# bluecube/minipath

Hardware: AMD Instinct MI355X
Metric: Mrays/s (higher is better)
Workload: dtype f32

## Files before the change

### minipath_amd/csrc/kernels.hip

```cpp
#include <hip/hip_runtime.h>

#include <algorithm>
#include <cfloat>
#include <cmath>
#include <cstdlib>
#include <type_traits>

#include "launch_plan.h"
#include "mp_internal.h"
#include "family_launch.h"
#include "ray_math.h"

#ifdef MP_PROF_MISSES
namespace mp {
namespace {
__device__ unsigned long long g_prof[8];
}
}
#define MP_PROF_COUNT(i) do { if ((threadIdx.x & 63u) == 0u) atomicAdd(&g_prof[i], 1ull); } while (0)
#endif
#include "mask_cache.h"
#include "group_walk.h"

namespace mp {
namespace {

struct RenderParams {
    DevScene scene;
    RayGen gen;
    const mp_block* tiles;
    uint32_t n_tiles, tile_size;
    float* out;
    uint32_t* counter;
    float inv_spp;
    uint32_t s_begin, s_end;
    uint32_t carry_in;
    uint32_t finalize;
    uint32_t chunked;
    const uint32_t* tile_order;
    unsigned long long* tile_cost;
    uint32_t lds_per_wave;
    uint32_t max_depth;
    unsigned long long* segments;
    float* pool;
    uint32_t pool_stride;
};

constexpr uint32_t kSumChunk = 256;
__device__ __forceinline__ void pixel_state_load(const RenderParams& P, size_t off, bool inpix, bool writer, float& acc, float& cnt) {
    acc = 0.0f;
    cnt = 0.0f;
    if (P.carry_in && inpix) {
        const float4 prev = *reinterpret_cast<const float4*>(P.out + off);
        acc = prev.x;
        cnt = P.chunked ? prev.y : prev.w;
    } else if (P.chunked && inpix && writer) {
        *reinterpret_cast<double*>(P.out + off + 2) = 0.0;
    }
}
__device__ __forceinline__ void chunk_flush(const RenderParams& P, size_t off, bool writer, float& acc) {
    if (writer) {
        double* t = reinterpret_cast<double*>(P.out + off + 2);
        *t = *t + static_cast<double>(acc);
    }
    acc = 0.0f;
}
__device__ __forceinline__ void pixel_state_store(const RenderParams& P, size_t off, float acc, float cnt) {
    if (P.chunked) {
        if (!P.finalize) {
            *reinterpret_cast<float2*>(P.out + off) = make_float2(acc, cnt);
            return;
        }
// ... 284 lines not shown
                const bool det_ok = fabsf(det) <= kHuge;
                const float xu = det_ok ? as_f(as_u(un) ^ det_sign) : 1.0f;
                if (__ballot(!(xu <= thr)) == 0) return;
                const float qx = fms(sy, e1z, sz * e1y), qy = fms(sz, e1x, sx * e1z), qz = fms(sx, e1y, sy * e1x);
                const float vn = fma_dot(r.dx, r.dy, r.dz, qx, qy, qz);
                const float tn = fma_dot(e2x, e2y, e2z, qx, qy, qz);
                const float xv = det_ok ? as_f(as_u(vn) ^ det_sign) : 1.0f, xt = det_ok ? as_f(as_u(tn) ^ det_sign) : 1.0f;
                if (__ballot(!(fminf(fminf(xu, xv), xt) <= thr)) == 0) return;
                const float inv_det = 1.0f / det;
                const float u = inv_det * un, v = inv_det * vn, t = inv_det * tn;
                const bool acc = (u >= 0.0f) & (v >= 0.0f) & ((u + v) <= 1.0f) & (t >= 0.0f) & (t < lim);
                best_t = acc ? t : best_t;
                lim = acc ? t : lim;
                bu = acc ? u : bu;
                bv = acc ? v : bv;
                bprim = acc ? tri : bprim;
                changed |= __ballot(acc);
            };
            float a0 = tp[0], a1 = tp[1], a2 = tp[2], a3 = tp[3], a4 = tp[4], a5 = tp[5], a6 = tp[6], a7 = tp[7], a8 = tp[8];
            uint32_t tri = first * 8u;
            for (uint32_t p = n_real >> 1; p > 0; p--) {
                const float b0 = tp[9], b1 = tp[10], b2 = tp[11], b3 = tp[12], b4 = tp[13], b5 = tp[14], b6 = tp[15], b7 = tp[16], b8 = tp[17];
                test(a0, a1, a2, a3, a4, a5, a6, a7, a8, tri);
                a0 = tp[18]; a1 = tp[19]; a2 = tp[20]; a3 = tp[21]; a4 = tp[22]; a5 = tp[23]; a6 = tp[24]; a7 = tp[25]; a8 = tp[26];
                test(b0, b1, b2, b3, b4, b5, b6, b7, b8, tri + 1u);
                tri += 2u;
                tp += 2 * kTriDwords;
            }
            if (n_real & 1u) test(a0, a1, a2, a3, a4, a5, a6, a7, a8, tri);
            if (changed != 0) stale_top = sp;
        }
    }
    hit.t = best_t; hit.u = bu; hit.v = bv; hit.prim = bprim;
}

struct RegStack3 {
    int ent, mlo, mhi;
    __device__ __forceinline__ RegStack3() : ent(0), mlo(0), mhi(0) {}
    __device__ __forceinline__ void push(int sp, uint32_t e, uint64_t m) {
        asm volatile("s_mov_b32 m0, %3\n\ts_nop 0\n\t"
                     "v_writelane_b32 %0, %4, m0\n\tv_writelane_b32 %1, %5, m0\n\tv_writelane_b32 %2, %6, m0"
                     : "+v"(ent), "+v"(mlo), "+v"(mhi)
                     : "s"(sp), "s"(e), "s"(static_cast<uint32_t>(m)), "s"(static_cast<uint32_t>(m >> 32))
                     : "m0");
    }
    __device__ __forceinline__ void pop(int sp, uint32_t& e, uint64_t& m) const {
        e = static_cast<uint32_t>(__builtin_amdgcn_readlane(ent, sp));
        m = static_cast<uint32_t>(__builtin_amdgcn_readlane(mlo, sp)) |
            (static_cast<uint64_t>(static_cast<uint32_t>(__builtin_amdgcn_readlane(mhi, sp))) << 32);
    }
};

template <int OCT>
__device__ __noinline__ uint32_t unit_list_slow(const float* __restrict__ nodes_pk, uint32_t* mcache, uint32_t node, uint32_t slots) {
    return unit_list_build(reinterpret_cast<const float4*>(nodes_pk), mcache, node, slots,
                           [](const float* b, const float bmn[3], const float bmx[3]) { return bounds_may_hit<OCT>(b, bmn, bmx); });
}
template <int OCT>
__device__ __forceinline__ bool trace_packet_cached(const DevScene& sc, const Ray& r, bool active, PacketHit& hit, uint32_t* mcache) {
    static_assert(kNullLink == MP_LINK_NULL, "mask_cache.h's copy of the null link");
    kfp nodes = (kfp)(uintptr_t)sc.nodes_pk;
    kfp tris = (kfp)(uintptr_t)sc.tris_aos;
    float best_t = FLT_MAX, bu = 0.0f, bv = 0.0f;
    uint32_t bprim = kNoPrim;
    RegStack3 st;
    int sp = 0;
    mcache[kRootListSlot] = sc.pk_count * sc.pk_mask_bits;
    wave_lds_sync();
    uint32_t cur = (static_cast<uint32_t>(kRootListSlot) << 16) | 1u;
    uint64_t pm = __ballot(active);
    for (;;) {
        if ((cur & 0xFFFFu) == 0u) {
            if (sp == 0) break;
            sp--;
            st.pop(sp, cur, pm);
        }
        cur -= 1u;
        const uint32_t src = __builtin_amdgcn_readfirstlane(mcache[(cur >> 16) + (cur & 0xFFFFu)]);
#ifndef MP_NO_EMPTY_SKIP
        if (static_cast<int32_t>(src) < 0) {
            MP_PROF_COUNT(7);
            continue;
        }
#endif
        const bool pon = __builtin_amdgcn_inverse_ballot_w64(pm);
        const krec8 rec = *reinterpret_cast<const __attribute__((address_space(4))) krec8*>(reinterpret_cast<const __attribute__((address_space(4))) char*>(nodes) + scalar_u(src * 32u));
        float t1, t2;
        slab<false, OCT>(rec[0], rec[1], rec[2], rec[3], rec[4], rec[5], r, pon ? best_t : -1.0f, t1, t2);
        const bool ok = t1 <= t2;
        if (__ballot(ok) == 0) continue;
        const uint32_t link = uniform_u(rec[6]);
        float lim = ok ? best_t : -1.0f;
        if ((link & 63u) == 0u) {
            MP_PROF_COUNT(2);
            const uint32_t node = link >> 6;
            const uint32_t slot = node_slot(node);
            const uint32_t tag = __builtin_amdgcn_readfirstlane(mcache[static_cast<uint32_t>(kMaskCacheHeader) + slot]);
            uint32_t list = __builtin_amdgcn_readfirstlane(mcache[static_cast<uint32_t>(kNodeListBase) + slot]);
            if (__builtin_expect(tag != node, 0)) {
                MP_PROF_COUNT(0);
                if (tag != 0xFFFFFFFFu) MP_PROF_COUNT(4);
                list = __builtin_amdgcn_readfirstlane(unit_list_slow<OCT>(sc.nodes_pk, mcache, node, sc.pk_mask_bits));
                if (list == kListOverflow) {
                    if (sp != 0 || (cur & 0xFFFFu) != 0u) {
                        MP_PROF_COUNT(6);
                        return false;
                    }
                    list = __builtin_amdgcn_readfirstlane(unit_list_slow<OCT>(sc.nodes_pk, mcache, node, sc.pk_mask_bits));
                }
            }
            if ((list & 0xFFFFu) != 0u) {
                if ((cur & 0xFFFFu) != 0u) {
                    st.push(sp, cur, pm);
                    sp++;
                }
                cur = list;
                pm = __ballot(lim >= 0.0f);
            }
        } else {
            const uint32_t first = link >> 6, n_real = link & 63u;
            kfp tp = tris + static_cast<size_t>(first) * (8 * kTriDwords);
            static_assert(kExitTiny == kTiny && kExitHuge == kHuge, "mask_cache.h's copies of the early-out constants");
            const float thr = lim >= 0.0f ? -kTiny : INFINITY;
            auto test = [&](const float v0x, const float v0y, const float v0z, const float e1x, const float e1y, const float e1z,
                            const float e2x, const float e2y, const float e2z, const uint32_t tri) {
                const float hx = fms(r.dy, e2z, r.dz * e2y), hy = fms(r.dz, e2x, r.dx * e2z), hz = fms(r.dx, e2y, r.dy * e2x);
                const float det = fma_dot(e1x, e1y, e1z, hx, hy, hz);
                const float sx = r.ox - v0x, sy = r.oy - v0y, sz = r.oz - v0z;
                const float un = fma_dot(sx, sy, sz, hx, hy, hz);
                const float xu = tri_flipped(det, un);
                if (__ballot(!(tri_exit1_key(det, xu) <= thr)) == 0) return;
                const float qx = fms(sy, e1z, sz * e1y), qy = fms(sz, e1x, sx * e1z), qz = fms(sx, e1y, sy * e1x);
                const float vn = fma_dot(r.dx, r.dy, r.dz, qx, qy, qz);
                const float tn = fma_dot(e2x, e2y, e2z, qx, qy, qz);
                const float xv = tri_flipped(det, vn), xt = tri_flipped(det, tn);
                if (__ballot(!(tri_exit2_key(det, xu, xv, xt) <= thr)) == 0) return;
                constexpr uint32_t kRcpLo = 0x10800000u , kRcpHi = 0x7E000000u ;
                const uint32_t wkey = (as_u(det) << 1) - (kRcpLo << 1);
                const float inv_det = __ballot(wkey > ((kRcpHi - kRcpLo) << 1)) == 0 ? rm::rcp_short(det) : 1.0f / det;
                const float u = inv_det * un, v = inv_det * vn, t = inv_det * tn;
                const bool acc = !(fminf(fminf(u, v), t) < 0.0f) & ((u + v) <= 1.0f) & (t < lim);
                best_t = acc ? t : best_t;
                lim = acc ? t : lim;
                bu = acc ? u : bu;
                bv = acc ? v : bv;
                bprim = acc ? tri : bprim;
            };
            const uint32_t ls = first & static_cast<uint32_t>(kLeafCacheEntries - 1);
            const uint32_t tag = mcache[kLeafTagBase + ls];
            const uint2 tm = reinterpret_cast<const uint2*>(mcache + kLeafMaskBase)[ls];
            uint64_t todo;
            if (__builtin_expect(__builtin_amdgcn_readfirstlane(tag) == first, 1)) {
                todo = __builtin_amdgcn_readfirstlane(tm.x) | (static_cast<uint64_t>(__builtin_amdgcn_readfirstlane(tm.y)) << 32);
            } else {
                MP_PROF_COUNT(1);
                const uint64_t m = leaf_mask_slow(sc.tris_aos, mcache, first, n_real);
                todo = __builtin_amdgcn_readfirstlane(static_cast<uint32_t>(m)) | (static_cast<uint64_t>(__builtin_amdgcn_readfirstlane(static_cast<uint32_t>(m >> 32))) << 32);
            }
#ifndef MP_NO_EMPTY_SKIP
            if (todo == 0 && (cur >> 16) != static_cast<uint32_t>(kRootListSlot)) {
                if ((threadIdx.x & 63u) == 0u) mcache[(cur >> 16) + (cur & 0xFFFFu)] = src | kEmptyLeafBit;
                wave_lds_sync();
            }
#endif
            if (todo != 0) {
                uint32_t c = static_cast<uint32_t>(__builtin_ctzll(todo));
                todo &= ~(1ull << c);
                kfp ta = tri_record(tp, c);
                krec8 ra = *reinterpret_cast<const __attribute__((address_space(4))) krec8*>(ta);
                float a8 = ta[8];
                while (todo != 0) {
                    const uint32_t cn = static_cast<uint32_t>(__builtin_ctzll(todo));
                    todo &= ~(1ull << cn);
                    kfp tb = tri_record(tp, cn);
                    const krec8 rb = *reinterpret_cast<const __attribute__((address_space(4))) krec8*>(tb);
                    const float b8 = tb[8];
                    test(ra[0], ra[1], ra[2], ra[3], ra[4], ra[5], ra[6], ra[7], a8, first * 8u + c);
                    ra = rb; a8 = b8;
                    c = cn;
                }
                test(ra[0], ra[1], ra[2], ra[3], ra[4], ra[5], ra[6], ra[7], a8, first * 8u + c);
            }
        }
    }
    hit.t = best_t; hit.u = bu; hit.v = bv; hit.prim = bprim;
    return true;
}

template <bool OCTANTS, class Stack, bool MC = false>
__device__ __forceinline__ void trace_packet(const DevScene& sc, const Ray& r, bool active, Stack& st, PacketHit& hit,
                                             const MaskCache& mc = MaskCache{nullptr}) {
    if (OCTANTS && MC) {
        if (__ballot(active & !mask_cache_ray_ok(r)) != 0) {
            const bool slow = active && (fabsf(r.ix) == INFINITY || fabsf(r.iy) == INFINITY || fabsf(r.iz) == INFINITY);
            if (__ballot(slow) != 0) trace_packet_impl<2, -1>(sc, r, active, st, hit);
            else trace_packet_impl<1, -1>(sc, r, active, st, hit);
            return;
        }
    } else {
        const bool slow = active && (fabsf(r.ix) == INFINITY || fabsf(r.iy) == INFINITY || fabsf(r.iz) == INFINITY);
        if (__ballot(slow) != 0) {
            trace_packet_impl<2, -1>(sc, r, active, st, hit);
            return;
        }
    }
    if (OCTANTS && sc.boxes_ordered) {
        const uint64_t am = __ballot(active);
        const uint64_t nx = __ballot(active && r.ix < 0.0f), ny = __ballot(active && r.iy < 0.0f), nz = __ballot(active && r.iz < 0.0f);
// ... 1524 lines not shown
    (void)hipFreeAsync(ws, st);
    return rc;
}

int launch_trace_rays(const DevScene& sc, const float* ox, const float* oy, const float* oz, const float* dx,
                      const float* dy, const float* dz, uint64_t n, const mp_hits_soa& hits, int cu_count, void* stream,
                      std::string& err) {
    return launch_rays(kQueryClosest, sc, ox, oy, oz, dx, dy, dz, nullptr, n, &hits, nullptr, cu_count, stream, err);
}

int launch_query_rays(const DevScene& sc, const float* ox, const float* oy, const float* oz, const float* dx, const float* dy,
                      const float* dz, const float* tmax, uint64_t n, const mp_hits_soa* hits, uint8_t* occluded, int cu_count,
                      void* stream, std::string& err) {
    return launch_rays(occluded ? kQueryAnyHit : kQueryBounded, sc, ox, oy, oz, dx, dy, dz, tmax, n, hits, occluded, cu_count, stream, err);
}

int launch_set_u64(unsigned long long* d_ptr, unsigned long long value, void* stream, std::string& err) {
    return launch(K_SET_U64, 1, 1, 0, static_cast<hipStream_t>(stream), err, d_ptr, value);
}

int launch_generate_rays(const mp_camera_sampler& s, uint32_t width, uint32_t spp, uint64_t seed, mp_block block,
                         uint32_t sample, float* ox, float* oy, float* oz, float* dx, float* dy, float* dz, void* stream,
                         std::string& err) {
    const uint64_t n = static_cast<uint64_t>(block.max_x - block.min_x) * (block.max_y - block.min_y);
    if (n == 0) return MP_OK;
    RayGen G;
    fill_raygen(G, s, width, spp, seed);
    const uint32_t grid = static_cast<uint32_t>(std::min<uint64_t>((n + 255) / 256, 8192));
    return launch(K_GENERATE_RAYS, grid, 256, 0, static_cast<hipStream_t>(stream), err, G, block, sample, ox, oy, oz, dx, dy, dz);
}

int launch_untile(uint32_t width, uint32_t height, uint32_t tile_size, const mp_block* d_tiles, uint32_t n_tiles,
                  const float* d_tiles_f32, float* d_image_f32, uint8_t* d_image_u8, void* stream, std::string& err,
                  uint32_t preview_mode, uint32_t preview_samples) {
    const uint64_t n = static_cast<uint64_t>(tile_size) * tile_size * n_tiles;
    if (n == 0) return MP_OK;
    const uint32_t grid = static_cast<uint32_t>(std::min<uint64_t>((n + 255) / 256, 8192));
    const uint32_t k = std::max<uint32_t>(preview_samples, 1u);
    return launch(K_UNTILE, grid, 256, 0, static_cast<hipStream_t>(stream), err, width, height, tile_size, d_tiles, n_tiles, d_tiles_f32,
                  d_image_f32, d_image_u8, preview_mode, 1.0f / static_cast<float>(k), 1.0 / static_cast<double>(k));
}

int launch_quantise(const float* d_rgba_f32, uint8_t* d_rgba_u8, uint64_t n_pixels, void* stream, std::string& err) {
    if (n_pixels == 0) return MP_OK;
    const uint32_t grid = static_cast<uint32_t>(std::min<uint64_t>((n_pixels + 255) / 256, 8192));
    return launch(K_QUANTISE, grid, 256, 0, static_cast<hipStream_t>(stream), err, d_rgba_f32, d_rgba_u8, n_pixels);
}

}

#ifdef MP_PROF_MISSES
extern "C" int mp_prof_read8(unsigned long long* out, int reset) {
    if (hipMemcpyFromSymbol(out, HIP_SYMBOL(mp::g_prof), sizeof(unsigned long long) * 8) != hipSuccess) return 1;
    if (reset) { unsigned long long z[8] = {0, 0, 0, 0, 0, 0, 0, 0}; if (hipMemcpyToSymbol(HIP_SYMBOL(mp::g_prof), z, sizeof(z)) != hipSuccess) return 1; }
    return 0;
}
extern "C" int mp_prof_read(unsigned long long* out, int reset) {
    unsigned long long all[8];
    if (mp_prof_read8(all, reset) != 0) return 1;
    for (int i = 0; i < 4; i++) out[i] = all[i];
    return 0;
}
#endif
```

### minipath_amd/csrc/mask_cache.h

```cpp
#pragma once

#include <hip/hip_runtime.h>

#include <cfloat>
#include <cmath>
#include <cstdint>

#include "camera_rays.h"

#ifndef MP_PROF_COUNT
#define MP_PROF_COUNT(i) do { } while (0)
#endif

namespace mp {
namespace mc {
__device__ __forceinline__ float as_f(uint32_t u) { return __uint_as_float(u); }
__device__ __forceinline__ uint32_t as_u(float f) { return __float_as_uint(f); }

__device__ __forceinline__ void wave_lds_sync() {
    __builtin_amdgcn_fence(__ATOMIC_RELEASE, "wavefront");
    __builtin_amdgcn_wave_barrier();
    __builtin_amdgcn_fence(__ATOMIC_ACQUIRE, "wavefront");
}

// ... 184 lines not shown
        for (int k = 0; k < 3; k++) pmax[g][k] = pmin[g][k];
        wave_min3_max3(pmin[g], pmax[g]);
    }
    float* hdr = reinterpret_cast<float*>(mc.lds);
    if (lane == 63) {
#pragma unroll
        for (int g = 0; g < 3; g++) {
#pragma unroll
            for (int k = 0; k < 3; k++) {
                const float lo = pmin[g][k], hi = pmax[g][k];
                const float pad = (hi - lo) * MP_MCACHE_MARGIN;
                float wlo = lo - pad, whi = hi + pad;
                if (g == 1) {
                    if ((wlo < 0.0f) != (lo < 0.0f) || wlo == 0.0f) wlo = lo;
                    if ((whi < 0.0f) != (hi < 0.0f) || whi == 0.0f) whi = hi;
                    if (!(fabsf(wlo) < INFINITY)) wlo = lo;
                    if (!(fabsf(whi) < INFINITY)) whi = hi;
                } else {
                    const float cap = g == 0 ? 2.0f * kCoordCap : 2.0f;
                    wlo = fmaxf(wlo, -cap); whi = fminf(whi, cap);
                }
                hdr[hdr_lo(g) + k] = wlo; hdr[hdr_lo(g) + 3 + k] = whi;
            }
        }
        mc.lds[kHdrState] = oct | 0x100u;
    }
    MP_PROF_COUNT(3);
#pragma unroll
    for (int i = 0; i < (kMaskCacheEntries + kLeafCacheEntries) / 64; i++) mc.lds[kMaskCacheHeader + i * 64 + lane] = 0xFFFFFFFFu;
    wave_lds_sync();
}
template <int OCT>
__device__ __forceinline__ bool bounds_may_hit(const float* b, const float bmn[3], const float bmx[3]) {
    float L[3], U[3];
#pragma unroll
    for (int k = 0; k < 3; k++) {
        const float y = bmn[k] - b[3 + k], z = bmx[k] - b[k];
        const float lo_src = ((OCT >> k) & 1) ? z : y, hi_src = ((OCT >> k) & 1) ? y : z;
        L[k] = fminf(lo_src * b[6 + k], lo_src * b[9 + k]);
        U[k] = fmaxf(hi_src * b[6 + k], hi_src * b[9 + k]);
    }
    const float t1 = fmaxf(fmaxf(L[0], 0.0f), fmaxf(L[1], L[2])), t2 = fminf(U[0], fminf(U[1], U[2]));
    return !(t1 > t2);
}

constexpr uint32_t kNullLink = 0xFFFFFFF8u;
constexpr uint32_t kListOverflow = 0xFFFFFFFFu;
constexpr uint32_t kEmptyLeafBit = 0x80000000u;
constexpr int kListDepth = 64;
__device__ __forceinline__ uint32_t node_slot(uint32_t node) {
    return min(node & static_cast<uint32_t>(kMaskCacheEntries - 1) & MP_NODE_SLOT_MASK, static_cast<uint32_t>(kMaskCacheEntries - 2));
}
template <class Kept>
__device__ __forceinline__ uint32_t unit_list_build(const float4* __restrict__ recs, uint32_t* mcache, uint32_t node, uint32_t slots, Kept kept) {
    const uint32_t lane = threadIdx.x & 63u;
    const float* b = reinterpret_cast<const float*>(mcache);
    node = __builtin_amdgcn_readfirstlane(node);
    slots = __builtin_amdgcn_readfirstlane(slots);
    auto kept_of = [&](uint32_t n, float4& c0, float4& c1) -> uint32_t {
        bool keep = false;
        c0 = make_float4(0.0f, 0.0f, 0.0f, 0.0f); c1 = c0;
        if (lane < slots) {
            const float4* r = recs + (static_cast<size_t>(n) * slots + lane) * 2;
            c0 = r[0]; c1 = r[1];
            const float bmn[3] = {c0.x, c0.y, c0.z}, bmx[3] = {c0.w, c1.x, c1.y};
            keep = as_u(c1.z) != kNullLink && kept(b, bmn, bmx);
        }
        return __builtin_amdgcn_readfirstlane(static_cast<uint32_t>(__ballot(keep)));
    };
    float4 c0, c1;
    uint32_t mask = kept_of(node, c0, c1);
    const uint32_t top = ~__builtin_amdgcn_readfirstlane(mcache[kArenaTopSlot]);
    if (top > static_cast<uint32_t>(kArenaEntries) || top + static_cast<uint32_t>(__popc(mask)) > static_cast<uint32_t>(kArenaEntries)) {
        MP_PROF_COUNT(5);
        wave_lds_sync();
#pragma unroll
        for (int i = 0; i < (kMaskCacheEntries + 63) / 64; i++)
            if (i * 64 + static_cast<int>(lane) < kMaskCacheEntries) mcache[kMaskCacheHeader + i * 64 + static_cast<int>(lane)] = 0xFFFFFFFFu;
        wave_lds_sync();
        return kListOverflow;
    }
    const uint32_t room = static_cast<uint32_t>(kArenaEntries) - top;
    uint32_t used = 0u, pend = static_cast<uint32_t>(__popc(mask)), cur = node;
    int st_node = 0, st_mask = 0, depth = 0;
    for (;;) {
        if (mask == 0u) {
            while (mask == 0u && depth > 0) {
                depth--;
                cur = static_cast<uint32_t>(__builtin_amdgcn_readlane(st_node, depth));
                mask = static_cast<uint32_t>(__builtin_amdgcn_readlane(st_mask, depth));
            }
            if (mask == 0u) break;
            if (lane < slots) {
                const float4* r = recs + (static_cast<size_t>(cur) * slots + lane) * 2;
                c0 = r[0]; c1 = r[1];
            }
        }
        const uint32_t j = static_cast<uint32_t>(__builtin_ctz(mask));
        mask &= mask - 1u;
        pend--;
        const uint32_t rec = cur * slots + j;
        auto from_lane = [&](float v) { return as_f(static_cast<uint32_t>(__builtin_amdgcn_readlane(static_cast<int>(as_u(v)), static_cast<int>(j)))); };
        const float4 p0 = make_float4(from_lane(c0.x), from_lane(c0.y), from_lane(c0.z), from_lane(c0.w));
        const float4 p1 = make_float4(from_lane(c1.x), from_lane(c1.y), from_lane(c1.z), 0.0f);
        const uint32_t link = as_u(p1.z);
        bool emit = true;
        if ((link & 63u) == 0u) {
            const uint32_t m = link >> 6;
            float4 g0, g1;
            const uint32_t km = kept_of(m, g0, g1);
            const bool sticks_out = ((km >> lane) & 1u) != 0u && lane < slots &&
                                    !(p0.x <= g0.x && p0.y <= g0.y && p0.z <= g0.z && g0.w <= p0.w && g1.x <= p1.x && g1.y <= p1.y);
            if (km == 0u) {
                emit = false;
            } else if (__ballot(sticks_out) == 0 && depth < kListDepth && used + pend + static_cast<uint32_t>(__popc(km)) <= room) {
                if (mask != 0u) {
                    asm volatile("s_mov_b32 m0, %2\n\ts_nop 0\n\tv_writelane_b32 %0, %3, m0\n\tv_writelane_b32 %1, %4, m0"
                                 : "+v"(st_node), "+v"(st_mask) : "s"(depth), "s"(__builtin_amdgcn_readfirstlane(cur)), "s"(__builtin_amdgcn_readfirstlane(mask)) : "m0");
                    depth++;
                }
                cur = m; mask = km; pend += static_cast<uint32_t>(__popc(km));
                c0 = g0; c1 = g1;
                emit = false;
            }
        }
        if (emit) {
            if (lane == 0u) mcache[static_cast<uint32_t>(kArenaBase) + top + used] = rec;
            used++;
        }
    }
    const uint32_t val = ((static_cast<uint32_t>(kArenaBase) + top) << 16) | used;
    if (lane == 0u) {
        const uint32_t slot = node_slot(node);
        mcache[static_cast<uint32_t>(kMaskCacheHeader) + slot] = node;
        mcache[static_cast<uint32_t>(kNodeListBase) + slot] = val;
        mcache[kArenaTopSlot] = ~(top + used);
    }
    wave_lds_sync();
    return val;
}

struct Iv {
    float lo, hi;
};
__device__ __forceinline__ Iv iv_neg(const Iv a) { return Iv{-a.hi, -a.lo}; }
__device__ __forceinline__ Iv iv_mul_c(const Iv a, const float c) {
    const float p = a.lo * c, q = a.hi * c;
    return Iv{fminf(p, q), fmaxf(p, q)};
}
__device__ __forceinline__ Iv iv_mul(const Iv a, const Iv b) {
    const float p1 = a.lo * b.lo, p2 = a.lo * b.hi, p3 = a.hi * b.lo, p4 = a.hi * b.hi;
    return Iv{fminf(fminf(p1, p2), fminf(p3, p4)), fmaxf(fmaxf(p1, p2), fmaxf(p3, p4))};
}
__device__ __forceinline__ Iv iv_fma_c(const Iv a, const float c, const Iv z) {
    return Iv{fminf(__builtin_fmaf(a.lo, c, z.lo), __builtin_fmaf(a.hi, c, z.lo)), fmaxf(__builtin_fmaf(a.lo, c, z.hi), __builtin_fmaf(a.hi, c, z.hi))};
}
__device__ __forceinline__ Iv iv_fma(const Iv a, const Iv b, const Iv z) {
    const float l1 = __builtin_fmaf(a.lo, b.lo, z.lo), l2 = __builtin_fmaf(a.lo, b.hi, z.lo), l3 = __builtin_fmaf(a.hi, b.lo, z.lo), l4 = __builtin_fmaf(a.hi, b.hi, z.lo);
    const float h1 = __builtin_fmaf(a.lo, b.lo, z.hi), h2 = __builtin_fmaf(a.lo, b.hi, z.hi), h3 = __builtin_fmaf(a.hi, b.lo, z.hi), h4 = __builtin_fmaf(a.hi, b.hi, z.hi);
    return Iv{fminf(fminf(l1, l2), fminf(l3, l4)), fmaxf(fmaxf(h1, h2), fmaxf(h3, h4))};
}
__device__ __forceinline__ bool tri_may_hit(const float* b, const float (&v0)[3], const float (&e1)[3], const float (&e2)[3]) {
    const Iv d[3] = {Iv{b[13], b[16]}, Iv{b[14], b[17]}, Iv{b[15], b[18]}};
    const Iv h[3] = {iv_fma_c(d[1], e2[2], iv_neg(iv_mul_c(d[2], e2[1]))), iv_fma_c(d[2], e2[0], iv_neg(iv_mul_c(d[0], e2[2]))),
                     iv_fma_c(d[0], e2[1], iv_neg(iv_mul_c(d[1], e2[0])))};
    const Iv det = iv_fma_c(h[2], e1[2], iv_fma_c(h[1], e1[1], iv_mul_c(h[0], e1[0])));
    if (!(det.lo > 0.0f || det.hi < 0.0f)) return true;
    const Iv inv = Iv{1.0f / det.hi, 1.0f / det.lo};
    if (!(fabsf(inv.lo) < INFINITY && fabsf(inv.hi) < INFINITY)) return true;
    const Iv s[3] = {Iv{b[0] - v0[0], b[3] - v0[0]}, Iv{b[1] - v0[1], b[4] - v0[1]}, Iv{b[2] - v0[2], b[5] - v0[2]}};
    const Iv u = iv_mul(inv, iv_fma(s[2], h[2], iv_fma(s[1], h[1], iv_mul(s[0], h[0]))));
    const Iv q[3] = {iv_fma_c(s[1], e1[2], iv_neg(iv_mul_c(s[2], e1[1]))), iv_fma_c(s[2], e1[0], iv_neg(iv_mul_c(s[0], e1[2]))),
                     iv_fma_c(s[0], e1[1], iv_neg(iv_mul_c(s[1], e1[0])))};
    const Iv v = iv_mul(inv, iv_fma(d[2], q[2], iv_fma(d[1], q[1], iv_mul(d[0], q[0]))));
    const Iv t = iv_mul(inv, iv_fma_c(q[2], e2[2], iv_fma_c(q[1], e2[1], iv_mul_c(q[0], e2[0]))));
    const bool miss = u.hi < 0.0f || v.hi < 0.0f || (u.lo + v.lo) > 1.0f || t.hi < 0.0f;
    return !miss;
}

constexpr float kExitTiny = 9.094947017729282e-13f;
constexpr float kExitHuge = 1099511627776.0f;
constexpr float kFarSlack = 1.00000095367431640625f;
__device__ __forceinline__ float tri_flipped(float det, float num) {
    return fabsf(det) <= kExitHuge ? as_f(as_u(num) ^ (as_u(det) & 0x80000000u)) : 1.0f;
}
__device__ __forceinline__ float tri_far_key(float det, float x) { return __builtin_fmaf(fabsf(det), kFarSlack, -x); }
__device__ __forceinline__ float tri_exit1_key(float det, float xu) {
#ifdef MP_NO_FAR_EXIT
    return xu;
#else
    return fminf(xu, tri_far_key(det, xu));
#endif
}
__device__ __forceinline__ float tri_exit2_key(float det, float xu, float xv, float xt) {
    const float near_key = fminf(fminf(xu, xv), xt);
#ifdef MP_NO_FAR_EXIT
    return near_key;
#else
    return fminf(fminf(near_key, tri_far_key(det, xu)), tri_far_key(det, xu + xv));
#endif
}

}
}
```

### minipath_amd/csrc/mask_probe.hip

```cpp
#include <hip/hip_runtime.h>

#include <cfloat>
#include <cstdint>

#include "mask_cache.h"

namespace {

using namespace mp::mc;

constexpr int kCounters = 8;
constexpr float kOrgCap = 2.0f * kCoordCap;

__device__ __forceinline__ uint64_t mix64(uint64_t z) {
    z = (z ^ (z >> 30)) * 0xbf58476d1ce4e5b9ull;
    z = (z ^ (z >> 27)) * 0x94d049bb133111ebull;
    return z ^ (z >> 31);
}
__device__ __forceinline__ uint64_t hsh(uint64_t seed, uint64_t c, uint32_t k) { return mix64(seed ^ mix64(c * 0x10000ull + k)); }
__device__ __forceinline__ float unit(uint64_t h) { return static_cast<float>(static_cast<uint32_t>(h >> 40)) * 0x1p-24f; }

__device__ __forceinline__ void record_case(unsigned long long* out, bool bad, uint64_t idx, bool hit, bool rejected, bool edge_only) {
    if ((threadIdx.x & 63) != 0) return;
    atomicAdd(out + 1, 1ull);
// ... 573 lines not shown
    if (unit >= n) return;
    uint32_t* const base = lds + w * kMaskCacheDwords;
    if (lane < static_cast<uint32_t>(kMaskCacheHeader)) base[lane] = static_cast<uint32_t>(hsh(0x0E17ull, unit, lane));
    constexpr int kTags = kLeafMaskBase - kMaskCacheHeader;
    for (int i = 0; i < kTags / 64; i++) base[kMaskCacheHeader + i * 64 + static_cast<int>(lane)] = static_cast<uint32_t>(i * 64) + lane;
    wave_lds_sync();
    mask_cache_begin_unit(MaskCache{base}, cam.s, jitter_scale, blocks[4 * unit], blocks[4 * unit + 1], blocks[4 * unit + 2], blocks[4 * unit + 3]);
    wave_lds_sync();
    uint32_t cleared = 0u;
    for (int i = 0; i < kTags / 64; i++) cleared += static_cast<uint32_t>(__popcll(__ballot(base[kMaskCacheHeader + i * 64 + static_cast<int>(lane)] == 0xFFFFFFFFu)));
    if (lane < 19u) out[kUnitOut * unit + lane] = base[lane];
    if (lane == 19u) out[kUnitOut * unit + 19u] = cleared;
}

constexpr int kListOut = 4 + kArenaRoom;
template <int OCT>
__device__ __noinline__ uint32_t list_slow(const float4* __restrict__ recs, uint32_t* mcache, uint32_t node, uint32_t slots) {
    return unit_list_build(recs, mcache, node, slots,
                           [](const float* b, const float bmn[3], const float bmx[3]) { return bounds_may_hit<OCT>(b, bmn, bmx); });
}
__global__ void __launch_bounds__(256) list_kernel(const float4* recs, uint32_t slots, const uint32_t* headers, const uint32_t* cases, uint32_t n,
                                                   uint32_t* out) {
    __shared__ __align__(16) uint32_t lds[4 * kMaskCacheDwords];
    const uint32_t w = threadIdx.x >> 6, lane = threadIdx.x & 63u;
    const uint32_t c = blockIdx.x * 4u + w;
    if (c >= n) return;
    uint32_t* const base = lds + w * kMaskCacheDwords;
    for (uint32_t i = lane; i < static_cast<uint32_t>(kMaskCacheDwords); i += 64u)
        base[i] = i < static_cast<uint32_t>(kMaskCacheHeader) ? headers[32u * c + i] : i < static_cast<uint32_t>(kLeafMaskBase) ? 0xFFFFFFFFu : 0xDEAD0000u + i;
    wave_lds_sync();
    const uint32_t node = cases[2u * c], top0 = cases[2u * c + 1u];
    if (lane == 0u) base[kArenaTopSlot] = ~top0;
    wave_lds_sync();
    uint32_t val;
    switch (__builtin_amdgcn_readfirstlane(base[kHdrState]) & 7u) {
        case 0: val = list_slow<0>(recs, base, node, slots); break;
        case 1: val = list_slow<1>(recs, base, node, slots); break;
        case 2: val = list_slow<2>(recs, base, node, slots); break;
        case 3: val = list_slow<3>(recs, base, node, slots); break;
        case 4: val = list_slow<4>(recs, base, node, slots); break;
        case 5: val = list_slow<5>(recs, base, node, slots); break;
        case 6: val = list_slow<6>(recs, base, node, slots); break;
        default: val = list_slow<7>(recs, base, node, slots); break;
    }
    wave_lds_sync();
    uint32_t* const o = out + static_cast<size_t>(c) * kListOut;
    if (lane == 0u) {
        const uint32_t slot = node_slot(node);
        o[0] = val; o[1] = ~base[kArenaTopSlot]; o[2] = base[static_cast<uint32_t>(kMaskCacheHeader) + slot]; o[3] = base[static_cast<uint32_t>(kNodeListBase) + slot];
    }
    for (uint32_t i = lane; i < static_cast<uint32_t>(kArenaRoom); i += 64u) o[4u + i] = base[static_cast<uint32_t>(kArenaBase) + i];
}

template <class F>
int run(F launch, unsigned long long* host) {
    (void)hipGetLastError();
    unsigned long long* dev = nullptr;
    unsigned long long init[kCounters] = {0ull, 0ull, ~0ull, 0ull, 0ull, 0ull, 0ull, 0ull};
    hipError_t e = hipMalloc(&dev, sizeof(init));
    if (e != hipSuccess) return static_cast<int>(e);
    e = hipMemcpy(dev, init, sizeof(init), hipMemcpyHostToDevice);
    if (e == hipSuccess) {
        launch(dev);
        e = hipGetLastError();
        if (e == hipSuccess) e = hipDeviceSynchronize();
        if (e == hipSuccess) e = hipMemcpy(host, dev, sizeof(init), hipMemcpyDeviceToHost);
    }
    const hipError_t ef = hipFree(dev);
    return static_cast<int>(e != hipSuccess ? e : ef);
}
void merge(unsigned long long* acc, const unsigned long long* r) {
    for (int i = 0; i < kCounters; i++) if (i != 2) acc[i] += r[i];
    if (r[2] < acc[2]) acc[2] = r[2];
}
void reset(unsigned long long* acc) {
    for (int i = 0; i < kCounters; i++) acc[i] = 0ull;
    acc[2] = ~0ull;
}
constexpr uint64_t kCasesPerLaunch = 1ull << 20;

template <class K>
int run_cases(K kernel, uint64_t seed, uint64_t ncases, uint32_t* dump_dev, unsigned long long* out) {
    unsigned long long acc[kCounters];
    reset(acc);
    for (uint64_t c0 = 0; c0 < ncases; c0 += kCasesPerLaunch) {
        const uint64_t n = ncases - c0 < kCasesPerLaunch ? ncases - c0 : kCasesPerLaunch;
        unsigned long long r[kCounters];
        if (int rc = run([&](unsigned long long* d) {
                hipLaunchKernelGGL(kernel, dim3(static_cast<uint32_t>((n + 3) / 4)), dim3(256), 0, 0, seed, c0, c0 + n, d, dump_dev);
            }, r))
            return rc;
        merge(acc, r);
    }
    for (int i = 0; i < kCounters; i++) out[i] = acc[i];
    return 0;
}

}

extern "C" {
int mp_mask_probe_tri(uint64_t seed, uint64_t ncases, unsigned long long* out) { return run_cases(tri_kernel, seed, ncases, nullptr, out); }
int mp_mask_probe_exits(uint64_t seed, uint64_t ncases, unsigned long long* out) { return run_cases(exit_kernel, seed, ncases, nullptr, out); }
int mp_mask_probe_box(uint64_t seed, uint64_t ncases, unsigned long long* out) { return run_cases(box_kernel, seed, ncases, nullptr, out); }
int mp_mask_probe_dump_dwords() { return kDumpCase; }
int mp_mask_probe_dump(int kind, uint64_t seed, uint64_t ncases, uint32_t* host, unsigned long long* out) {
    (void)hipGetLastError();
// ... 63 lines not shown
    const float* p = sampler;
    for (int k = 0; k < 3; k++) { cam.s.center[k] = p[k]; cam.s.up[k] = p[3 + k]; cam.s.right[k] = p[6 + k]; cam.s.film_origin_offset[k] = p[9 + k]; }
    cam.s.pixel_scale = p[12]; cam.s.lens_radius = p[13]; cam.s.lens_weight = p[14];
    uint32_t *dblocks = nullptr, *dout = nullptr;
    hipError_t e = hipMalloc(&dblocks, sizeof(uint32_t) * 4u * n);
    if (e == hipSuccess) e = hipMalloc(&dout, sizeof(uint32_t) * kUnitOut * n);
    if (e == hipSuccess) e = hipMemcpy(dblocks, blocks, sizeof(uint32_t) * 4u * n, hipMemcpyHostToDevice);
    if (e == hipSuccess) {
        hipLaunchKernelGGL(unit_kernel, dim3((n + 3u) / 4u), dim3(256), 0, 0, cam, jitter_scale, dblocks, n, dout);
        e = hipGetLastError();
        if (e == hipSuccess) e = hipDeviceSynchronize();
        if (e == hipSuccess) e = hipMemcpy(out, dout, sizeof(uint32_t) * kUnitOut * n, hipMemcpyDeviceToHost);
    }
    (void)hipFree(dblocks);
    (void)hipFree(dout);
    return static_cast<int>(e);
}
int mp_mask_probe_pass(uint64_t seed, uint64_t nwaves, unsigned long long* out) {
    return run([&](unsigned long long* d) {
        hipLaunchKernelGGL(pass_kernel, dim3(static_cast<uint32_t>(nwaves / 4)), dim3(256), 0, 0, seed, d);
    }, out);
}
int mp_mask_probe_list_dwords() { return kListOut; }
int mp_mask_probe_list(const uint32_t* recs, uint32_t n_nodes, uint32_t slots, const uint32_t* headers, const uint32_t* cases, uint32_t ncases,
                       uint32_t* out, uint32_t* info) {
    (void)hipGetLastError();
    if (info) { info[0] = static_cast<uint32_t>(kArenaEntries); info[1] = static_cast<uint32_t>(kMaskCacheEntries); info[2] = static_cast<uint32_t>(kArenaBase); }
    if (slots != 8u && slots != 16u) return -1;
    for (uint32_t c = 0; c < ncases; c++)
        if (cases[2u * c] >= n_nodes || cases[2u * c + 1u] > static_cast<uint32_t>(kArenaEntries)) return -1;
    for (size_t i = 0; i < static_cast<size_t>(n_nodes) * slots; i++) {
        const uint32_t link = recs[i * 8u + 6u];
        if (link != kNullLink && (link & 63u) == 0u && (link >> 6) >= n_nodes) return -1;
    }
    if (ncases == 0u) return 0;
    uint32_t *drecs = nullptr, *dhdr = nullptr, *dcases = nullptr, *dout = nullptr;
    const size_t rec_bytes = sizeof(uint32_t) * 8u * slots * n_nodes, out_bytes = sizeof(uint32_t) * kListOut * static_cast<size_t>(ncases);
    hipError_t e = hipMalloc(&drecs, rec_bytes);
    if (e == hipSuccess) e = hipMalloc(&dhdr, sizeof(uint32_t) * 32u * ncases);
    if (e == hipSuccess) e = hipMalloc(&dcases, sizeof(uint32_t) * 2u * ncases);
    if (e == hipSuccess) e = hipMalloc(&dout, out_bytes);
    if (e == hipSuccess) e = hipMemcpy(drecs, recs, rec_bytes, hipMemcpyHostToDevice);
    if (e == hipSuccess) e = hipMemcpy(dhdr, headers, sizeof(uint32_t) * 32u * ncases, hipMemcpyHostToDevice);
    if (e == hipSuccess) e = hipMemcpy(dcases, cases, sizeof(uint32_t) * 2u * ncases, hipMemcpyHostToDevice);
    if (e == hipSuccess) {
        hipLaunchKernelGGL(list_kernel, dim3((ncases + 3u) / 4u), dim3(256), 0, 0, reinterpret_cast<const float4*>(drecs), slots, dhdr, dcases, ncases, dout);
        e = hipGetLastError();
        if (e == hipSuccess) e = hipDeviceSynchronize();
        if (e == hipSuccess) e = hipMemcpy(out, dout, out_bytes, hipMemcpyDeviceToHost);
    }
    (void)hipFree(drecs); (void)hipFree(dhdr); (void)hipFree(dcases); (void)hipFree(dout);
    return static_cast<int>(e);
}
}
```

Before: 37850.

## Batch-fill leaf triangle masks eagerly when building a node's unit list

When a node's unit list is rebuilt on a cache miss and it contains at least two leaves, the leaf triangle masks for all its leaves are computed together. Triangles from several leaves are packed across the 64 lanes, tested against the packet bounds in one pass, and written into the leaf mask cache, with empty leaves marked in the list. This replaces many later per-leaf lazy misses that each use only a few lanes. The cost is extra work at list build time for leaves that may never be visited, and possible eviction of useful leaf-cache entries. Probe kernels and profiling counters are also added.

```diff
diff --git a/minipath_amd/csrc/kernels.hip b/minipath_amd/csrc/kernels.hip
--- a/minipath_amd/csrc/kernels.hip
+++ b/minipath_amd/csrc/kernels.hip
@@ -14,10 +14,11 @@
 #ifdef MP_PROF_MISSES
 namespace mp {
 namespace {
-__device__ unsigned long long g_prof[8];
+__device__ unsigned long long g_prof[10];
 }
 }
 #define MP_PROF_COUNT(i) do { if ((threadIdx.x & 63u) == 0u) atomicAdd(&g_prof[i], 1ull); } while (0)
+#define MP_PROF_ADD(i, n) do { if ((threadIdx.x & 63u) == 0u) atomicAdd(&g_prof[i], (n)); } while (0)
 #endif
 #include "mask_cache.h"
 #include "group_walk.h"
@@ -408,13 +409,18 @@
 };
 
 template <int OCT>
-__device__ __noinline__ uint32_t unit_list_slow(const float* __restrict__ nodes_pk, uint32_t* mcache, uint32_t node, uint32_t slots) {
-    return unit_list_build(reinterpret_cast<const float4*>(nodes_pk), mcache, node, slots,
-                           [](const float* b, const float bmn[3], const float bmx[3]) { return bounds_may_hit<OCT>(b, bmn, bmx); });
+__device__ __noinline__ uint32_t unit_list_slow(const float* __restrict__ nodes_pk, const float* __restrict__ tris_aos, uint32_t* mcache, uint32_t node,
+                                                uint32_t slots) {
+    uint32_t leaf_entries = 0u;
+    const uint32_t list = unit_list_build(reinterpret_cast<const float4*>(nodes_pk), mcache, node, slots,
+                                          [](const float* b, const float bmn[3], const float bmx[3]) { return bounds_may_hit<OCT>(b, bmn, bmx); }, leaf_entries);
+    if (list != kListOverflow && leaf_entries >= kBatchMinLeaves) leaf_batch_fill(reinterpret_cast<const float4*>(nodes_pk), tris_aos, mcache, list);
+    return list;
 }
 template <int OCT>
 __device__ __forceinline__ bool trace_packet_cached(const DevScene& sc, const Ray& r, bool active, PacketHit& hit, uint32_t* mcache) {
     static_assert(kNullLink == MP_LINK_NULL, "mask_cache.h's copy of the null link");
+    static_assert(kTriRecDwords == kTriDwords, "mask_cache.h's copy of the triangle record's size");
     kfp nodes = (kfp)(uintptr_t)sc.nodes_pk;
     kfp tris = (kfp)(uintptr_t)sc.tris_aos;
     float best_t = FLT_MAX, bu = 0.0f, bv = 0.0f;
@@ -456,13 +462,13 @@
             if (__builtin_expect(tag != node, 0)) {
                 MP_PROF_COUNT(0);
                 if (tag != 0xFFFFFFFFu) MP_PROF_COUNT(4);
-                list = __builtin_amdgcn_readfirstlane(unit_list_slow<OCT>(sc.nodes_pk, mcache, node, sc.pk_mask_bits));
+                list = __builtin_amdgcn_readfirstlane(unit_list_slow<OCT>(sc.nodes_pk, sc.tris_aos, mcache, node, sc.pk_mask_bits));
                 if (list == kListOverflow) {
                     if (sp != 0 || (cur & 0xFFFFu) != 0u) {
                         MP_PROF_COUNT(6);
                         return false;
                     }
-                    list = __builtin_amdgcn_readfirstlane(unit_list_slow<OCT>(sc.nodes_pk, mcache, node, sc.pk_mask_bits));
+                    list = __builtin_amdgcn_readfirstlane(unit_list_slow<OCT>(sc.nodes_pk, sc.tris_aos, mcache, node, sc.pk_mask_bits));
                 }
             }
             if ((list & 0xFFFFu) != 0u) {
@@ -510,6 +516,7 @@
                 todo = __builtin_amdgcn_readfirstlane(tm.x) | (static_cast<uint64_t>(__builtin_amdgcn_readfirstlane(tm.y)) << 32);
             } else {
                 MP_PROF_COUNT(1);
+                MP_PROF_COUNT(9);
                 const uint64_t m = leaf_mask_slow(sc.tris_aos, mcache, first, n_real);
                 todo = __builtin_amdgcn_readfirstlane(static_cast<uint32_t>(m)) | (static_cast<uint64_t>(__builtin_amdgcn_readfirstlane(static_cast<uint32_t>(m >> 32))) << 32);
             }
@@ -2140,7 +2147,12 @@
 #ifdef MP_PROF_MISSES
 extern "C" int mp_prof_read8(unsigned long long* out, int reset) {
     if (hipMemcpyFromSymbol(out, HIP_SYMBOL(mp::g_prof), sizeof(unsigned long long) * 8) != hipSuccess) return 1;
-    if (reset) { unsigned long long z[8] = {0, 0, 0, 0, 0, 0, 0, 0}; if (hipMemcpyToSymbol(HIP_SYMBOL(mp::g_prof), z, sizeof(z)) != hipSuccess) return 1; }
+    if (reset) { unsigned long long z[10] = {0, 0, 0, 0, 0, 0, 0, 0, 0, 0}; if (hipMemcpyToSymbol(HIP_SYMBOL(mp::g_prof), z, sizeof(z)) != hipSuccess) return 1; }
+    return 0;
+}
+extern "C" int mp_prof_read10(unsigned long long* out, int reset) {
+    if (hipMemcpyFromSymbol(out, HIP_SYMBOL(mp::g_prof), sizeof(unsigned long long) * 10) != hipSuccess) return 1;
+    if (reset) { unsigned long long z[10] = {0, 0, 0, 0, 0, 0, 0, 0, 0, 0}; if (hipMemcpyToSymbol(HIP_SYMBOL(mp::g_prof), z, sizeof(z)) != hipSuccess) return 1; }
     return 0;
 }
 extern "C" int mp_prof_read(unsigned long long* out, int reset) {
diff --git a/minipath_amd/csrc/mask_cache.h b/minipath_amd/csrc/mask_cache.h
--- a/minipath_amd/csrc/mask_cache.h
+++ b/minipath_amd/csrc/mask_cache.h
@@ -260,7 +260,7 @@
     return min(node & static_cast<uint32_t>(kMaskCacheEntries - 1) & MP_NODE_SLOT_MASK, static_cast<uint32_t>(kMaskCacheEntries - 2));
 }
 template <class Kept>
-__device__ __forceinline__ uint32_t unit_list_build(const float4* __restrict__ recs, uint32_t* mcache, uint32_t node, uint32_t slots, Kept kept) {
+__device__ __forceinline__ uint32_t unit_list_build(const float4* __restrict__ recs, uint32_t* mcache, uint32_t node, uint32_t slots, Kept kept, uint32_t& leaf_entries) {
     const uint32_t lane = threadIdx.x & 63u;
     const float* b = reinterpret_cast<const float*>(mcache);
     node = __builtin_amdgcn_readfirstlane(node);
@@ -289,6 +289,7 @@
         return kListOverflow;
     }
     const uint32_t room = static_cast<uint32_t>(kArenaEntries) - top;
+    leaf_entries = 0u;
     uint32_t used = 0u, pend = static_cast<uint32_t>(__popc(mask)), cur = node;
     int st_node = 0, st_mask = 0, depth = 0;
     for (;;) {
@@ -335,6 +336,7 @@
         if (emit) {
             if (lane == 0u) mcache[static_cast<uint32_t>(kArenaBase) + top + used] = rec;
             used++;
+            leaf_entries += (link & 63u) != 0u ? 1u : 0u;
         }
     }
     const uint32_t val = ((static_cast<uint32_t>(kArenaBase) + top) << 16) | used;
@@ -346,6 +348,12 @@
     }
     wave_lds_sync();
     return val;
+}
+
+template <class Kept>
+__device__ __forceinline__ uint32_t unit_list_build(const float4* __restrict__ recs, uint32_t* mcache, uint32_t node, uint32_t slots, Kept kept) {
+    uint32_t leaf_entries = 0u;
+    return unit_list_build(recs, mcache, node, slots, kept, leaf_entries);
 }
 
 struct Iv {
@@ -385,6 +393,78 @@
     const bool miss = u.hi < 0.0f || v.hi < 0.0f || (u.lo + v.lo) > 1.0f || t.hi < 0.0f;
     return !miss;
 }
+constexpr int kTriRecDwords = 9;
+
+#ifdef MP_NO_EMPTY_SKIP
+constexpr bool kMarkAtBuild = false;
+#else
+constexpr bool kMarkAtBuild = true;
+#endif
+#ifndef MP_PROF_ADD
+#define MP_PROF_ADD(i, n) do { } while (0)
+#endif
+constexpr uint32_t kBatchMinLeaves = 2u;
+template <class T>
+__device__ __forceinline__ T* uniform_p(T* p) {
+    const uint64_t v = reinterpret_cast<uint64_t>(p);
+    const uint32_t lo = __builtin_amdgcn_readfirstlane(static_cast<uint32_t>(v)), hi = __builtin_amdgcn_readfirstlane(static_cast<uint32_t>(v >> 32));
+    return reinterpret_cast<T*>((static_cast<uint64_t>(hi) << 32) | lo);
+}
+__device__ __forceinline__ void leaf_batch_fill(const float4* __restrict__ recs_, const float* __restrict__ tris_aos_, uint32_t* mcache_, uint32_t list) {
+    const float* recs = uniform_p(reinterpret_cast<const float*>(recs_));
+    const float* tris_aos = uniform_p(tris_aos_);
+    uint32_t* mcache = uniform_p(mcache_);
+    list = __builtin_amdgcn_readfirstlane(list);
+    const uint32_t base = list >> 16, n = list & 0xFFFFu;
+    for (uint32_t e0 = 0u; e0 < n; e0 += 64u) {
+        uint32_t link = 0u;
+        if (e0 + (threadIdx.x & 63u) < n) {
+            const uint32_t ent = mcache[base + e0 + (threadIdx.x & 63u)] & ~kEmptyLeafBit;
+            link = as_u(recs[static_cast<size_t>(ent) * 8u + 6u]);
+            if (link == kNullLink) link = 0u;
+            if ((link & 63u) == 0u) link = 0u;
+        }
+        uint64_t leaves = __ballot(link != 0u);
+        while (leaves != 0) {
+            uint32_t total = 0u, my_tri = 0u;
+            uint64_t bm = 0;
+            do {
+                const uint32_t k = static_cast<uint32_t>(__builtin_ctzll(leaves));
+                const uint32_t lk = static_cast<uint32_t>(__builtin_amdgcn_readlane(static_cast<int>(link), static_cast<int>(k)));
+                const uint32_t c = lk & 63u;
+                if (total + c > 64u) break;
+                const uint32_t rel = (threadIdx.x & 63u) - total;
+                if (rel < c) my_tri = (lk >> 6) * 8u + rel;
+                total += c;
+                bm |= 1ull << k;
+                leaves &= leaves - 1ull;
+            } while (leaves != 0);
+            bool keep = false;
+            if ((threadIdx.x & 63u) < total) {
+                const float* tv = tris_aos + static_cast<size_t>(my_tri) * kTriRecDwords;
+                const float v0[3] = {tv[0], tv[1], tv[2]}, e1[3] = {tv[3], tv[4], tv[5]}, e2[3] = {tv[6], tv[7], tv[8]};
+                keep = tri_may_hit(reinterpret_cast<const float*>(mcache), v0, e1, e2);
+            }
+            const uint64_t m = __ballot(keep);
+            MP_PROF_COUNT(8);
+            MP_PROF_ADD(1, static_cast<unsigned long long>(__popcll(bm)));
+            uint32_t at = 0u;
+            for (uint64_t w = bm; w != 0; w &= w - 1ull) {
+                const uint32_t k = static_cast<uint32_t>(__builtin_ctzll(w));
+                const uint32_t lk = static_cast<uint32_t>(__builtin_amdgcn_readlane(static_cast<int>(link), static_cast<int>(k)));
+                const uint32_t c = lk & 63u, first = lk >> 6, ls = first & static_cast<uint32_t>(kLeafCacheEntries - 1);
+                const uint64_t bits = (m >> at) & ((1ull << c) - 1ull);
+                at += c;
+                if ((threadIdx.x & 63u) == 0u) {
+                    mcache[kLeafTagBase + ls] = first;
+                    reinterpret_cast<uint2*>(mcache + kLeafMaskBase)[ls] = make_uint2(static_cast<uint32_t>(bits), static_cast<uint32_t>(bits >> 32));
+                    if (kMarkAtBuild && bits == 0ull) mcache[base + e0 + k] |= kEmptyLeafBit;
+                }
+            }
+        }
+    }
+    wave_lds_sync();
+}
 
 constexpr float kExitTiny = 9.094947017729282e-13f;
 constexpr float kExitHuge = 1099511627776.0f;
diff --git a/minipath_amd/csrc/mask_probe.hip b/minipath_amd/csrc/mask_probe.hip
--- a/minipath_amd/csrc/mask_probe.hip
+++ b/minipath_amd/csrc/mask_probe.hip
@@ -649,6 +649,67 @@
     for (uint32_t i = lane; i < static_cast<uint32_t>(kArenaRoom); i += 64u) o[4u + i] = base[static_cast<uint32_t>(kArenaBase) + i];
 }
 
+constexpr int kBatchOut = 4 + kArenaRoom + 3 * kLeafCacheEntries + 2 * kArenaRoom;
+__device__ __noinline__ void batch_slow(const float4* __restrict__ recs, const float* __restrict__ tris_aos, uint32_t* mcache, uint32_t list) {
+    leaf_batch_fill(recs, tris_aos, mcache, list);
+}
+__device__ __noinline__ uint64_t lazy_slow(const float* __restrict__ tris_aos, uint32_t* mcache, uint32_t first, uint32_t n_real) {
+    const uint32_t j = threadIdx.x & 63u;
+    bool keep = false;
+    if (j < n_real) {
+        const float* tv = tris_aos + (static_cast<size_t>(first) * 8 + j) * kTriRecDwords;
+        const float v0[3] = {tv[0], tv[1], tv[2]}, e1[3] = {tv[3], tv[4], tv[5]}, e2[3] = {tv[6], tv[7], tv[8]};
+        keep = tri_may_hit(reinterpret_cast<const float*>(mcache), v0, e1, e2);
+    }
+    return __ballot(keep);
+}
+__global__ void __launch_bounds__(64) batch_kernel(const float4* recs, uint32_t slots, const float* tris_aos, const uint32_t* headers, const uint32_t* cases,
+                                                   const uint32_t* entries, uint32_t n, uint32_t* out) {
+    __shared__ __align__(16) uint32_t lds[kMaskCacheDwords];
+    const uint32_t lane = threadIdx.x & 63u;
+    const uint32_t c = blockIdx.x;
+    if (c >= n) return;
+    uint32_t* const base = lds;
+    for (uint32_t i = lane; i < static_cast<uint32_t>(kMaskCacheDwords); i += 64u)
+        base[i] = i < static_cast<uint32_t>(kMaskCacheHeader) ? headers[32u * c + i] : i < static_cast<uint32_t>(kLeafMaskBase) ? 0xFFFFFFFFu : 0xDEAD0000u + i;
+    wave_lds_sync();
+    const uint32_t node = __builtin_amdgcn_readfirstlane(cases[2u * c]), n_hand = __builtin_amdgcn_readfirstlane(cases[2u * c + 1u]);
+    uint32_t list;
+    if (node != 0xFFFFFFFFu) {
+        switch (__builtin_amdgcn_readfirstlane(base[kHdrState]) & 7u) {
+            case 0: list = list_slow<0>(recs, base, node, slots); break;
+            case 1: list = list_slow<1>(recs, base, node, slots); break;
+            case 2: list = list_slow<2>(recs, base, node, slots); break;
+            case 3: list = list_slow<3>(recs, base, node, slots); break;
+            case 4: list = list_slow<4>(recs, base, node, slots); break;
+            case 5: list = list_slow<5>(recs, base, node, slots); break;
+            case 6: list = list_slow<6>(recs, base, node, slots); break;
+            default: list = list_slow<7>(recs, base, node, slots); break;
+        }
+        list = __builtin_amdgcn_readfirstlane(list);
+    } else {
+        for (uint32_t i = lane; i < n_hand; i += 64u) base[static_cast<uint32_t>(kArenaBase) + i] = entries[static_cast<size_t>(c) * kArenaRoom + i];
+        if (lane == 0u) base[kArenaTopSlot] = ~n_hand;
+        list = (static_cast<uint32_t>(kArenaBase) << 16) | n_hand;
+        wave_lds_sync();
+    }
+    uint32_t* const o = out + static_cast<size_t>(c) * kBatchOut;
+    const uint32_t n_ent = list == kListOverflow ? 0u : list & 0xFFFFu, first_dw = list >> 16;
+    if (list != kListOverflow) batch_slow(recs, tris_aos, base, list);
+    wave_lds_sync();
+    if (lane == 0u) { o[0] = list; o[1] = n_ent; o[2] = 0u; o[3] = 0u; }
+    for (uint32_t i = lane; i < static_cast<uint32_t>(kArenaRoom); i += 64u) o[4u + i] = base[static_cast<uint32_t>(kArenaBase) + i];
+    for (uint32_t i = lane; i < 3u * static_cast<uint32_t>(kLeafCacheEntries); i += 64u) o[4u + kArenaRoom + i] = base[static_cast<uint32_t>(kLeafTagBase) + i];
+    uint32_t* const ol = o + 4 + kArenaRoom + 3 * kLeafCacheEntries;
+    for (uint32_t i = 0; i < n_ent && i < static_cast<uint32_t>(kArenaRoom); i++) {
+        const uint32_t ent = __builtin_amdgcn_readfirstlane(base[first_dw + i]) & ~kEmptyLeafBit;
+        const uint32_t link = __builtin_amdgcn_readfirstlane(as_u(reinterpret_cast<const float*>(recs)[static_cast<size_t>(ent) * 8u + 6u]));
+        uint64_t m = 0;
+        if (link != kNullLink && (link & 63u) != 0u) m = lazy_slow(tris_aos, base, link >> 6, link & 63u);
+        if (lane == 0u) { ol[2u * i] = static_cast<uint32_t>(m); ol[2u * i + 1u] = static_cast<uint32_t>(m >> 32); }
+    }
+}
+
 template <class F>
 int run(F launch, unsigned long long* host) {
     (void)hipGetLastError();
@@ -818,4 +879,49 @@
     (void)hipFree(drecs); (void)hipFree(dhdr); (void)hipFree(dcases); (void)hipFree(dout);
     return static_cast<int>(e);
 }
-}
+int mp_mask_probe_batch_dwords() { return kBatchOut; }
+int mp_mask_probe_batches(const uint32_t* recs, uint32_t n_nodes, uint32_t slots, const float* tris, uint32_t n_tris, const uint32_t* headers,
+                          const uint32_t* cases, const uint32_t* entries, uint32_t ncases, uint32_t* out, uint32_t* info) {
+    (void)hipGetLastError();
+    if (info) { info[0] = static_cast<uint32_t>(kArenaRoom); info[1] = static_cast<uint32_t>(kLeafCacheEntries); info[2] = kMarkAtBuild ? 1u : 0u; info[3] = static_cast<uint32_t>(kArenaEntries); }
+    if (slots != 8u && slots != 16u) return -1;
+    const size_t n_recs = static_cast<size_t>(n_nodes) * slots;
+    for (size_t i = 0; i < n_recs; i++) {
+        const uint32_t link = recs[i * 8u + 6u];
+        if (link == kNullLink) continue;
+        if ((link & 63u) == 0u) { if ((link >> 6) >= n_nodes) return -1; }
+        else if (static_cast<uint64_t>(link >> 6) * 8u + (link & 63u) > n_tris) return -1;
+    }
+    for (uint32_t c = 0; c < ncases; c++) {
+        const uint32_t node = cases[2u * c], n = cases[2u * c + 1u];
+        if (node != 0xFFFFFFFFu) { if (node >= n_nodes) return -1; continue; }
+        if (n > static_cast<uint32_t>(kArenaEntries)) return -1;
+        for (uint32_t i = 0; i < n; i++) if (entries[static_cast<size_t>(c) * kArenaRoom + i] >= n_recs) return -1;
+    }
+    if (ncases == 0u) return 0;
+    uint32_t *drecs = nullptr, *dhdr = nullptr, *dcases = nullptr, *dent = nullptr, *dout = nullptr;
+    float* dtris = nullptr;
+    const size_t rec_bytes = sizeof(uint32_t) * 8u * n_recs, tri_bytes = sizeof(float) * kTriRecDwords * (n_tris ? n_tris : 1u);
+    const size_t ent_bytes = sizeof(uint32_t) * kArenaRoom * static_cast<size_t>(ncases), out_bytes = sizeof(uint32_t) * kBatchOut * static_cast<size_t>(ncases);
+    hipError_t e = hipMalloc(&drecs, rec_bytes);
+    if (e == hipSuccess) e = hipMalloc(&dtris, tri_bytes);
+    if (e == hipSuccess) e = hipMalloc(&dhdr, sizeof(uint32_t) * 32u * ncases);
+    if (e == hipSuccess) e = hipMalloc(&dcases, sizeof(uint32_t) * 2u * ncases);
+    if (e == hipSuccess) e = hipMalloc(&dent, ent_bytes);
+    if (e == hipSuccess) e = hipMalloc(&dout, out_bytes);
+    if (e == hipSuccess) e = hipMemcpy(drecs, recs, rec_bytes, hipMemcpyHostToDevice);
+    if (e == hipSuccess && n_tris) e = hipMemcpy(dtris, tris, sizeof(float) * kTriRecDwords * n_tris, hipMemcpyHostToDevice);
+    if (e == hipSuccess) e = hipMemcpy(dhdr, headers, sizeof(uint32_t) * 32u * ncases, hipMemcpyHostToDevice);
+    if (e == hipSuccess) e = hipMemcpy(dcases, cases, sizeof(uint32_t) * 2u * ncases, hipMemcpyHostToDevice);
+    if (e == hipSuccess) e = hipMemcpy(dent, entries, ent_bytes, hipMemcpyHostToDevice);
+    if (e == hipSuccess) e = hipMemset(dout, 0, out_bytes);
+    if (e == hipSuccess) {
+        hipLaunchKernelGGL(batch_kernel, dim3(ncases), dim3(64), 0, 0, reinterpret_cast<const float4*>(drecs), slots, dtris, dhdr, dcases, dent, ncases, dout);
+        e = hipGetLastError();
+        if (e == hipSuccess) e = hipDeviceSynchronize();
+        if (e == hipSuccess) e = hipMemcpy(out, dout, out_bytes, hipMemcpyDeviceToHost);
+    }
+    (void)hipFree(drecs); (void)hipFree(dtris); (void)hipFree(dhdr); (void)hipFree(dcases); (void)hipFree(dent); (void)hipFree(dout);
+    return static_cast<int>(e);
+}
+}
```

After: 38060, median of 6. Within noise of the previous version (+0.6%).
